# pweigmann/harmonic-power-flow

Measured on AMD Instinct MI355X. Metric: NR iterations/sec + ms/iter, 1 000-bus x 25-harmonic feeder; |dV| vs reference, higher is better.
Workload: dtype f64

## Files before the change

harmonic-power-flow_amd/csrc/hpf_block.hip:

```cpp
#include <algorithm>
#include <chrono>
#include <complex>
#include <cstdio>
#include <cstdlib>
#include <functional>
#include <rocsolver/rocsolver.h>
#include <thread>

#include "hpf_internal.hpp"
#include "hpf_gj.hpp"
#include "hpf_blk_jobs.hpp"
#include "hpf_blk_invert_mfma.hpp"
#include "hpf_gj_dense.hpp"
#include "hpf_gj_mfma.hpp"

using namespace hpf;

#ifdef HPF_FACTOR_STAMPS
#define HPF_STAMP_DECL long long st0 = 0, st1 = 0, st2 = 0, st3 = 0, st4 = 0, st5 = 0, st6 = 0
#define HPF_STAMP(v) \
    if (ablate & 16) v = __builtin_amdgcn_s_memtime()
#else
#define HPF_STAMP_DECL
#define HPF_STAMP(v)
// ... 676 lines not shown
                       h->cur_s0, h->d_pivflag, h->piv_limit, ts);
    return launch_status(h);
}

int wave_block_size(int b) { return b <= 12 ? 12 : (b <= 28 ? 28 : (b <= 52 ? 52 : (b <= 100 ? 100 : 0))); }

size_t factor_lds_bytes(int b) { return gj_dense_lds_bytes(b); }

template <int R>
int launch_factor(hpf_handle* h, const TreeDev& T, const int* nodes, int count, const int* active) {
    ScopedTimer t(h, T_SOLVE);
    const int b = 2 * h->Hn;
    const size_t lds = factor_lds_bytes(b);
    if (lds > 64 * 1024) {
        if (lds > 160 * 1024) return HPF_E_ARG;
        const hipError_t ea = hipFuncSetAttribute(reinterpret_cast<const void*>(&k_tree_factor<R>), hipFuncAttributeMaxDynamicSharedMemorySize, (int)lds);
        if (ea != hipSuccess) {
            h->last_detail = (int)ea;
            return HPF_E_HIP;
        }
    }
    hipLaunchKernelGGL((k_tree_factor<R>), dim3((unsigned)count, (unsigned)h->cur_S), dim3(256), lds, h->cur_stream, h->M, T,
                       nodes, b, h->N, h->Nc, active, h->d_U, h->d_E, h->d_f, h->d_Z, h->d_w, h->cur_s0);
    return launch_status(h);
}


template <int B>
__global__ __launch_bounds__(256) void k_level_back(
    Model M, TreeDev T, const int* __restrict__ sl_nodes, int n_sl, const int* __restrict__ lf_nodes, int n_lf, const int* __restrict__ gj_nodes, int n_gj,
    int b, int N, int Nc, const int* __restrict__ active, int S_cnt, const double* __restrict__ Zall, const double* __restrict__ wall,
    double* __restrict__ xall, const double* __restrict__ Hall, const double* __restrict__ Minv, const double* __restrict__ lbimg,
    const double* __restrict__ sbimg, const double* __restrict__ lzimg, const double* __restrict__ lfK, const double* __restrict__ lfS, int s0) {
    static_assert(64 * ((B + 16) / 16) == 256, "k_level_back: blocks of 52 rows (four wavefronts in every body)");
    const int ytiles = (S_cnt + LB_SB - 1) / LB_SB;
    const int bid = (int)blockIdx.x;
#if HPF_BATCH_XCD
    const int nb_sl = ((n_sl + 7) / 8) * 8 * ytiles, nb_lf = ((n_lf + 7) / 8) * 8 * ytiles;
    if (bid < nb_sl) {
        const int t_ = bid >> 3, bx = (t_ / ytiles) * 8 + (bid & 7);
        if (bx >= n_sl) return;
        sleaf_back_batch_body<B>(bx, t_ % ytiles, M, sl_nodes, b, active, S_cnt, wall, xall, Hall, sbimg, lzimg, Zall, lfS, s0);
    } else if (bid < nb_sl + nb_lf) {
        const int i = bid - nb_sl, t_ = i >> 3, bx = (t_ / ytiles) * 8 + (i & 7);
        if (bx >= n_lf) return;
        leaf_back_batch_body<B>(bx, t_ % ytiles, M, lf_nodes, b, active, S_cnt, wall, xall, Hall, lbimg, lfK, lfS, s0);
    } else {
#else
    const int nb_sl = n_sl * ytiles, nb_lf = n_lf * ytiles;
    if (bid < nb_sl) {
        sleaf_back_batch_body<B>(bid % n_sl, bid / n_sl, M, sl_nodes, b, active, S_cnt, wall, xall, Hall, sbimg, lzimg, Zall, lfS, s0);
    } else if (bid < nb_sl + nb_lf) {
        const int i = bid - nb_sl;
        leaf_back_batch_body<B>(i % n_lf, i / n_lf, M, lf_nodes, b, active, S_cnt, wall, xall, Hall, lbimg, lfK, lfS, s0);
    } else {
#endif
        const int i = bid - nb_sl - nb_lf;
        back_q_body<B>(i % n_gj, i / n_gj, M, T, gj_nodes, b, N, Nc, active, Zall, wall, xall, (double*)nullptr, Hall, Minv, lfK, lfS, s0);
    }
}

template <int B>
int launch_level_back(hpf_handle* h, const TreeDev& T, const int* sl_nodes, int n_sl, const int* lf_nodes, int n_lf, const int* gj_nodes, int n_gj,
                      const int* active) {
    const Tree& tr = active_tree(h);
    const unsigned ytiles = (unsigned)((h->cur_S + LB_SB - 1) / LB_SB);
#if HPF_BATCH_XCD
    const unsigned grid = (unsigned)(((n_sl + 7) / 8) * 8 + ((n_lf + 7) / 8) * 8) * ytiles + (unsigned)n_gj * (unsigned)h->cur_S;
#else
    const unsigned grid = (unsigned)(n_sl + n_lf) * ytiles + (unsigned)n_gj * (unsigned)h->cur_S;
#endif
    if ((unsigned)(n_sl + n_lf) * ytiles + (unsigned)n_gj * (unsigned)h->cur_S == 0) return HPF_OK;
    hipLaunchKernelGGL((k_level_back<B>), dim3(grid), dim3(256), 0, h->cur_stream, h->M, T, sl_nodes, n_sl, lf_nodes, n_lf, gj_nodes, n_gj, 2 * h->Hn,
                       h->N, h->Nc, active, h->cur_S, h->d_Z, h->d_w, h->d_x, h->d_H, tr.d_Minv, tr.d_lbimg, tr.d_sbimg, tr.d_lzimg, h->d_lfK, h->d_lfS,
                       h->cur_s0);
    return launch_status(h);
}

template <int B>
__global__ __launch_bounds__(64 * ((B + 16) / 16)) void k_back_walk(
    Model M, TreeDev T, const int* __restrict__ recs, const int* __restrict__ slots, const int* __restrict__ list_ptr, int b, int N, int Nc,
    const int* __restrict__ active, const double* __restrict__ Zall, const double* __restrict__ wall, double* __restrict__ xall,
    const double* __restrict__ Hall, const double* __restrict__ Minv, const double* __restrict__ lfK, const double* __restrict__ lfS, int s0) {
    __shared__ double xl[WALK_SLOTS + 2][B];
    const int beg = list_ptr[blockIdx.x], end = list_ptr[blockIdx.x + 1], tid = threadIdx.x;
    if (beg >= end) return;
    BackQIn<B> cur, nxt;
    back_q_load<B>(cur, beg, blockIdx.y, M, T, recs, b, active, Zall, wall, Hall, Minv, s0);
    if (cur.s < 0) return;
    const double* xs = xall + (size_t)cur.s * M.n * B;
    for (int i = beg; i < end; ++i) {
        const int2 sl = reinterpret_cast<const int2*>(slots)[i];
        const int par = cur.kp.y, crole = cur.kp.w >> 28;
        if (tid < B) {
            if (par >= 0 && sl.x < 0) xl[WALK_SLOTS][tid] = xs[(size_t)par * B + tid];
            if (crole == 1 && sl.y < 0) xl[WALK_SLOTS + 1][tid] = xs[(size_t)T.comp_child[cur.kp.w & 0x0fffffff] * B + tid];
        }
        lds_barrier();
        if (i + 1 < end) back_q_load<B>(nxt, i + 1, blockIdx.y, M, T, recs, b, active, Zall, wall, Hall, Minv, s0);
        const double x = back_q_compute<B>(cur, M, T, b, N, Nc, xall, (double*)nullptr, lfK, lfS, xl[sl.x < 0 ? WALK_SLOTS : sl.x],
                                           xl[sl.y < 0 ? WALK_SLOTS + 1 : sl.y]);
        if (tid < B) xl[(i - beg) % WALK_SLOTS][tid] = x;
        lds_barrier();
        cur = nxt;
    }
}

template <int B>
int launch_back_walk(hpf_handle* h, const Tree& tr, const TreeDev& T, int list0, int count, const int* active) {
    constexpr int NT = (B + 16) / 16;
    hipLaunchKernelGGL((k_back_walk<B>), dim3((unsigned)count, (unsigned)h->cur_S), dim3(64 * NT), 0, h->cur_stream, h->M, T, tr.d_walk_rec,
                       tr.d_walk_slot, tr.d_walk_ptr + list0, 2 * h->Hn, h->N, h->Nc, active, h->d_Z, h->d_w, h->d_x, h->d_H, tr.d_Minv,
                       h->d_lfK, h->d_lfS, h->cur_s0);
    return launch_status(h);
}

__global__ __launch_bounds__(256) void k_border_prepare(int n, int Hn, int Bst, int b, int r, int v0, int vfirst, const int* __restrict__ tb_bus,
                                                        int n_tb, const double* __restrict__ g, cplx* __restrict__ U, cplx* __restrict__ E,
                                                        cplx* __restrict__ I0, double* __restrict__ fb) {
    const int j = blockIdx.y, v = vfirst + j;
    const size_t dst = (size_t)(v0 + j);
    const int t = blockIdx.x * 256 + threadIdx.x;
    if (t < n * Hn) {
        U[dst * n * Hn + t] = U[(size_t)r * n * Hn + t];
        E[dst * n * Hn + t] = E[(size_t)r * n * Hn + t];
    }
    if (t < n) I0[dst * n + t] = I0[(size_t)r * n + t];
    if (t < n * Bst) {
        double val = 0.0;
        if (v == 0) {
            val = fb[(size_t)r * n * Bst + t];
            if (g) {
                const int bus = t / Bst, l = t - bus * Bst;
                if (l < b)
                    for (int a = 0; a < n_tb; ++a)
                        if (tb_bus[a] == bus) val -= g[a * b + l];
            }
        } else {
            const int a = (v - 1) / b, l = (v - 1) - a * b;
            if (t == tb_bus[a] * Bst + l) val = 1.0;
        }
        fb[dst * n * Bst + t] = val;
    }
}

__global__ __launch_bounds__(256) void k_border_build(Model M, int Bst, int b, int r, int v0, int vfirst, int m, const int* __restrict__ tb_bus,
                                                      const int* __restrict__ tb_ptr, const int* __restrict__ tb_adj,
                                                      const cplx* __restrict__ Uall, const cplx* __restrict__ Eall,
                                                      const double* __restrict__ xall, double* __restrict__ bM, double* __restrict__ brhs) {
    const int row = blockIdx.x * 256 + threadIdx.x;
    const int col = vfirst + blockIdx.y;
    if (row >= m) return;
    const int a = row / b, l = row - a * b, q = l >> 1, t = l & 1;
    const int i = tb_bus[a];
    const size_t so = (size_t)r * M.n * M.Hn;
    const double* x = xall + (size_t)(v0 + blockIdx.y) * M.n * Bst;
    double acc = 0.0;
    for (int e = tb_ptr[a]; e < tb_ptr[a + 1]; ++e) {
        const int j = tb_adj[3 * e], ent = tb_adj[3 * e + 1];
        double g4[4];
        coupling_block(M, Uall + so, Eall + so, q, i, j, ent, g4);
        acc = fma(g4[t * 2], x[(size_t)j * Bst + 2 * q], acc);
        acc = fma(g4[t * 2 + 1], x[(size_t)j * Bst + 2 * q + 1], acc);
    }
    if (col == 0)
        brhs[row] = acc;
    else
        bM[(size_t)(col - 1) * m + row] = acc + (row == col - 1 ? 1.0 : 0.0);
}

__global__ __launch_bounds__(256) void k_border_finish(int count, int r, int v0, int nv, double* __restrict__ xall, int* __restrict__ pivflag) {
    const int t = blockIdx.x * 256 + threadIdx.x;
    if (t < count) xall[(size_t)r * count + t] = xall[(size_t)v0 * count + t];
    if (t < nv && pivflag[v0 + t]) {
        atomicOr(pivflag + r, pivflag[v0 + t]);
        pivflag[v0 + t] = 0;
    }
}

}

#include "hpf_tree_plan.hpp"

namespace hpf {

static int level_batched(const hpf_handle* h, const Tree& T, int l, int* kind) {
    int nbatch = (l == 0 && h->sw.leafbatch && h->has_ctree && T.lvl_all_leaf[0]) ? T.n_lazy_level0 : 0;
// ... 986 lines not shown
```

harmonic-power-flow_amd/csrc/hpf_internal.hpp:

```cpp
#pragma once
#include <hip/hip_runtime.h>
#include <rocblas/rocblas.h>
#include <stdint.h>

#include <stdlib.h>
#include <string.h>

#include <string>
#include <vector>

#include "../../include/hpf.h"
#include "hpf_assembly.hpp"
#include "hpf_devmem.hpp"
#include "hpf_switches.hpp"

namespace hpf {

struct HipBackend {
    static constexpr int oom = (int)hipErrorOutOfMemory;
    static int alloc(void** p, size_t bytes) { return (int)hipMalloc(p, bytes); }
    static int free(void* p) { return (int)hipFree(p); }
    static int copy_in(void* dst, const void* src, size_t bytes) { return (int)hipMemcpy(dst, src, bytes, hipMemcpyHostToDevice); }
};
using DevMem = DevOwner<HipBackend>;

enum LinForm {
    LIN_ROOTS = 0,
    LIN_BUNDLE,
    LIN_TREE,
    LIN_LEVELS
};

enum { T_MISMATCH = 0, T_JACOBIAN = 1, T_SOLVE = 2, T_UPDATE = 3, T_BACK = 4, T_GJ = 5, T_GJ_DEV = 6, T_RESID = 7, T_COUNT = 8 };

struct TimedSpan {
    int which;
    hipEvent_t e0, e1;
};

#ifndef HPF_WALK_SLOTS
#define HPF_WALK_SLOTS 32
#endif
constexpr int WALK_LISTS = 8, WALK_SLOTS = HPF_WALK_SLOTS;
static_assert(WALK_SLOTS >= 2, "the walk's ring holds at least the previous bus");
constexpr int TAIL_SLOTS = 2;

struct Tree {
    int n_levels = 0;
    int n_depths = 0;
    std::vector<int> parent;
    std::vector<int> lvl_ptr;
    std::vector<int> lvl_nodes;
    std::vector<int> dep_ptr;
    std::vector<int> dep_nodes;
    std::vector<int> child_ptr;
    std::vector<int> child;
    std::vector<int> child_mid;
    std::vector<int> lin;
    std::vector<int> lin_ptr;
    std::vector<int> lin_post;
    std::vector<int> all_ptr, all_post;
    int n_lin_roots = 0;
    int n_dense = 0;
    int* d_parent = nullptr;
    int* d_lvl_nodes = nullptr;
    int* d_dep_nodes = nullptr;
    int* d_child_ptr = nullptr;
    int* d_child = nullptr;
    int* d_e_up = nullptr;
    int* d_e_dn = nullptr;
    int* d_child_mid = nullptr;
    int* d_lin = nullptr;
    int* d_lin_ptr = nullptr;
    int* d_lin_post = nullptr;
    int* d_all_ptr = nullptr;
    int* d_all_post = nullptr;
    int* d_fdesc = nullptr;
    int* d_child3 = nullptr;
    int* d_bdesc = nullptr;
    int n_chains = 0;
    std::vector<int> chain_ptr, chain_nodes, chain_ch;
    int* d_dchild = nullptr;
    int* d_chain_ptr = nullptr;
    int* d_chain_nodes = nullptr;
    int* d_chain_ch = nullptr;
    int n_lin_heights = 0;
    std::vector<int> lh_ptr;
    int* d_lrec = nullptr;
    int n_lin_bundles2 = 0, lin_np = 0;
    int lin_maxunit = 0;
    int* d_lb2rec = nullptr;
    int* d_lb2x = nullptr;
    int* d_lb2ptr = nullptr;
    int chains_bundled = 0;
    int* d_lb2cptr = nullptr;
    int* d_lb2clist = nullptr;
    int n_lin_bundles = 0;
    LinForm lin_form = LIN_ROOTS;
    bool chain_launches = false;
    int* d_lbrec = nullptr;
    int* d_lbptr = nullptr;
    int* d_crec = nullptr;
    int* d_cnode = nullptr;
    int n_all_heights = 0;
    std::vector<int> ah_ptr;
    int* d_arec = nullptr;
    std::vector<int> lvl_all_leaf;
    std::vector<int> toff_tab;
    std::vector<char> plain_gj;
    int n_cleaf = 0;
    double* d_Minv = nullptr;
    int n_lazy_parents = 0, n_lazy_leaves = 0;
    int n_lazy_level0 = 0;
    std::vector<int> lvl_nbatch;
    std::vector<int> dep_nleaf;
    std::vector<int> dep_nskip;
    int census[8] = {0, 0, 0, 0, 0, 0, 0, 0};
    std::vector<int> bsleaf_ptr;
    int n_bsleaf = 0;
    int* d_bsleaf = nullptr;
    double* d_sbimg = nullptr;
    std::vector<int> bsl_dep_ptr, bleaf_dep_ptr;
    int* d_bsleaf_dep = nullptr;
    int n_bleaf = 0;
    int* d_bleaf = nullptr;
    double* d_lbimg = nullptr;
    int* d_lzrec = nullptr;
// ... 252 lines not shown
```

harmonic-power-flow_amd/csrc/hpf_quad.hpp:

```cpp
#pragma once

template <int CTRL>
__device__ __forceinline__ double dpp_f64(double v) {
    int lo = __double2loint(v), hi = __double2hiint(v);
    lo = __builtin_amdgcn_update_dpp(lo, lo, CTRL, 0xf, 0xf, false);
    hi = __builtin_amdgcn_update_dpp(hi, hi, CTRL, 0xf, 0xf, false);
    return __hiloint2double(hi, lo);
}

__device__ __forceinline__ double row_sum16(double v) {
    v += dpp_f64<0xB1>(v);
    v += dpp_f64<0x4E>(v);
    v += dpp_f64<0x141>(v);
    v += dpp_f64<0x140>(v);
    return v;
}

__device__ __forceinline__ Blk2 blk_current(cplx y, cplx Uj, cplx Ej) {
    Blk2 b;
    b.dV = cmul_unf(y, Ej);
    b.dA = cmul_unf(cmulj(y), Uj);
    return b;
}
__device__ __forceinline__ Blk2 blk_current_diag(cplx y, cplx U, cplx E, cplx yn, bool nonlinear) {
    Blk2 b = blk_current(y, U, E);
    if (nonlinear) {
        b.dV = csub(b.dV, cmul_unf(yn, E));
        b.dA = csub(b.dA, cmul_unf(cmulj(yn), U));
    }
    return b;
}
__device__ __forceinline__ Blk2 blk_power_off(cplx y, cplx Ui, cplx Uj, cplx Ej) {
    const cplx yu = cmul_unf(y, Uj);
    const cplx ye = cmul_unf(y, Ej);
    Blk2 b;
    b.dV = cmul_unf(Ui, cconj(ye));
    b.dA = cmul_unf(cmulj(Ui), cconj(cneg(yu)));
    return b;
}
__device__ __forceinline__ Blk2 blk_power_diag(cplx y, cplx U, cplx E, cplx I) {
    const cplx yu = cmul_unf(y, U);
    const cplx ye = cmul_unf(y, E);
    Blk2 b;
    b.dV = cadd(cmul_unf(E, cconj(I)), cmul_unf(U, cconj(ye)));
    b.dA = cmul_unf(cmulj(U), cconj(csub(I, yu)));
    return b;
}
__device__ __forceinline__ void mask_block(int n, int c, int q, int i, int j, const Blk2& blk, double out[4]) {
#pragma unroll
    for (int tr = 0; tr < 2; ++tr)
#pragma unroll
        for (int tc = 0; tc < 2; ++tc)
            out[tr * 2 + tc] = (loc_valid(n, c, i, 2 * q + tr) && loc_valid(n, c, j, 2 * q + tc)) ? pick(blk, tr, tc) : 0.0;
}

template <int B>
struct TileIO {
    static constexpr int NT = (B + 16) / 16;
    static constexpr int LW = (B + 1 - 16 * (NT - 1)) <= 8 ? 8 : 16;
    static constexpr int RG = (NT - 1) * 64 + 4 * LW;
    static constexpr int NE = B / 4, NP = NE / 2;
    static_assert(NE == 2 * NP + 1, "odd number of row groups");
    __device__ static __forceinline__ size_t off2(int p, int wv, int lg, int jj) {
        return (size_t)p * 2 * RG + (wv < NT - 1 ? wv * 128 + (lg * 16 + jj) * 2 : (NT - 1) * 128 + (lg * LW + jj) * 2);
    }
    __device__ static __forceinline__ size_t off1(int wv, int lg, int jj) {
        return (size_t)NP * 2 * RG + (wv < NT - 1 ? wv * 64 + lg * 16 + jj : (NT - 1) * 64 + lg * LW + jj);
    }
    __device__ static __forceinline__ size_t off(int tr, int reg, int wv, int lg, int jj) {
        const int e = tr * 4 + reg;
        return e < 2 * NP ? off2(e >> 1, wv, lg, jj) + (e & 1) : off1(wv, lg, jj);
    }
    __device__ static __forceinline__ bool ok(int wv, int jj) { return wv < NT - 1 || jj < LW; }
    __device__ static __forceinline__ void load(const double* base, int wv, int lg, int jj, double (&v)[NT * 4]) {
        const bool in = ok(wv, jj);
#pragma unroll
        for (int p = 0; p < NP; ++p) {
            double2 t = {0.0, 0.0};
            if (in) t = *reinterpret_cast<const double2*>(base + off2(p, wv, lg, jj));
            v[2 * p] = t.x;
            v[2 * p + 1] = t.y;
        }
        v[NE - 1] = in ? base[off1(wv, lg, jj)] : 0.0;
    }
    __device__ static __forceinline__ void store(double* base, int wv, int lg, int jj, const double (&v)[NT * 4]) {
        if (!ok(wv, jj)) return;
#pragma unroll
        for (int p = 0; p < NP; ++p) *reinterpret_cast<double2*>(base + off2(p, wv, lg, jj)) = double2{v[2 * p], v[2 * p + 1]};
        base[off1(wv, lg, jj)] = v[NE - 1];
    }
};

template <int NT>
__device__ __forceinline__ void lz_aop(const double* p, double (&a)[NT]) {
    if constexpr (NT % 2 == 0) {
#pragma unroll
        for (int t2 = 0; t2 < NT / 2; ++t2) {
            const double2 v = *reinterpret_cast<const double2*>(p + 2 * t2);
            a[2 * t2] = v.x;
            a[2 * t2 + 1] = v.y;
        }
    } else {
#pragma unroll
        for (int t = 0; t < NT; ++t) a[t] = p[t];
    }
}

#define HPF_WAVE_LDS_FENCE() asm volatile("s_waitcnt lgkmcnt(0)" ::: "memory")

#ifndef HPF_LEAF_XCD
#define HPF_LEAF_XCD 1
#endif
#ifndef HPF_Q100L_OCC
#define HPF_Q100L_OCC 2
#endif
#ifndef HPF_Q100_OCC
#define HPF_Q100_OCC 2
#endif
#ifndef HPF_Q_OCC
#define HPF_Q_OCC 4
#endif

template <int B>
struct FqLds {
    static constexpr int NT = (B + 16) / 16, RP = 16 * NT > 64 ? 16 * NT : 64;
    cplx* ynl;
    double* tab;
    double* dgb;
    double (*cc)[RP * 3];
    double (*panel)[NT * 64];
    double (*wl)[16];
    double (*pv)[16];
    double* gl;
    double* hl;
    double* slb;
    double* gl2;
    double* hl2;
    double* pbuf;
    __device__ __forceinline__ static FqLds carve(double* smem_) {
        FqLds L;
        L.ynl = reinterpret_cast<cplx*>(smem_);
        L.tab = smem_ + 2 * (B / 2) * (B / 2);
        L.dgb = L.tab + (B / 2) * 8;
        L.cc = reinterpret_cast<double (*)[RP * 3]>(L.dgb + RP * 3);
        L.panel = reinterpret_cast<double (*)[NT * 64]>(L.dgb + RP * 3 + NT * RP * 3);
        L.wl = reinterpret_cast<double (*)[16]>(L.dgb + RP * 3 + NT * RP * 3 + 2 * NT * 64);
        L.pv = reinterpret_cast<double (*)[16]>(L.dgb + RP * 3 + NT * RP * 3 + 2 * NT * 64 + 32);
        L.gl = L.dgb + RP * 3 + NT * RP * 3 + 2 * NT * 64 + 64;
        L.hl = L.gl + NT * 32;
        L.slb = L.hl + NT * 32;
        L.gl2 = B <= 52 ? L.slb : L.slb + 2;
        L.hl2 = L.gl2 + NT * 32;
        L.pbuf = smem_;
        return L;
    }
};

template <int B>
constexpr int factor_q_lds() {
    constexpr int NT = (B + 16) / 16, RP = 16 * NT > 64 ? 16 * NT : 64;
    return (B / 2) * 8 + RP * 3 + NT * RP * 3 + 2 * NT * 64 + 32 + 32 + NT * 32 + NT * 32 + 2 * (B / 2) * (B / 2) +
           (B <= 52 ? 2 * B * 10 + 200 + 4 : 2 + 2 * NT * 32);
}
static_assert(factor_q_lds<52>() >= 52 * 53 && factor_q_lds<28>() >= 28 * 29 && factor_q_lds<12>() >= 12 * 13 && factor_q_lds<100>() >= 64 * 101,
              "dense-push buffer of a compress step fits the factor body's LDS");

// ... 1131 lines not shown
    double* __restrict__ lfK, double* __restrict__ lfS, long long* __restrict__ dbg, int ablate, int s0,
    int* __restrict__ pivflag, double piv_limit, unsigned long long* __restrict__ tstamp, int leaf_count, unsigned leaf_S) {
    constexpr int NT = (B + 16) / 16, RP = 16 * NT > 64 ? 16 * NT : 64;
    FqLds<B> lds;
    if constexpr (LEAF) {
        __shared__ cplx ynl[(B / 2) * (B / 2)];
        __shared__ double tab[(B / 2) * 8], dgb[RP * 3], cc[NT][RP * 3], panel[2][NT * 64], wl[2][16], pv[2][16], gl[NT * 32], hl[NT * 32];
        __shared__ double slb[B <= 52 ? 2 * B * 10 + 200 + 4 : 1];
        lds.ynl = ynl; lds.tab = tab; lds.dgb = dgb; lds.cc = cc; lds.panel = panel; lds.wl = wl; lds.pv = pv; lds.gl = gl; lds.hl = hl; lds.slb = slb;
        lds.gl2 = lds.hl2 = lds.pbuf = nullptr;
    } else {
        __shared__ __attribute__((aligned(16))) double smem[factor_q_lds<B>()];
        lds = FqLds<B>::carve(smem);
    }
    int bx = blockIdx.x, by = blockIdx.y;
#if HPF_LEAF_XCD
    if constexpr (LEAF) {
        const unsigned id = blockIdx.x, t = id >> 3, S_ = gridDim.y == 1 ? leaf_S : 1u;
        by = (int)(t % S_);
        bx = (int)((t / S_) * 8u + (id & 7u));
        if (bx >= leaf_count) return;
    }
#endif
    factor_q_body<B, LEAF>(lds, bx, by, M, T, nodes, b, N, Nc, active, Uall, Eall, fall, Zall, wall, linAall, Call, Hall, I0all, chG,
                           chH, chD, chy, Minv, lfK, lfS, dbg, ablate, s0, pivflag, piv_limit, tstamp);
}

__device__ __forceinline__ void lds_barrier() {
    __builtin_amdgcn_fence(__ATOMIC_RELEASE, "workgroup", "local");
    __builtin_amdgcn_s_barrier();
    __builtin_amdgcn_fence(__ATOMIC_ACQUIRE, "workgroup", "local");
}

template <int B>
struct BackQIn {
    static constexpr int NT = (B + 16) / 16;
    int4 kp;
    int s;
    double x;
    double zr[NT * 4];
    double hk0, hk1, h20, h21;
};

template <int B>
__device__ __forceinline__ void back_q_load(
    BackQIn<B>& in, const int bx_, const int by_, const Model& M, const TreeDev& T, const int* __restrict__ nodes, int b,
    const int* __restrict__ active, const double* __restrict__ Zall, const double* __restrict__ wall, const double* __restrict__ Hall,
    const double* __restrict__ Minv, int s0) {
    constexpr int NT = (B + 16) / 16;
    constexpr size_t CT = (size_t)NT * NT * 256;
    const int s = active ? active[by_ + s0] : (int)by_ + s0;
    in.s = s;
    if (s < 0) return;
    const int4 kp = reinterpret_cast<const int4*>(nodes)[bx_];
    in.kp = kp;
    const int k = kp.x, par = kp.y, cleaf = kp.z;
    const int crole = kp.w >> 28, cinfo = kp.w & 0x0fffffff;
    const int tid = threadIdx.x, lane = tid & 63, lg = lane >> 4, jj = lane & 15;
    const int wv = __builtin_amdgcn_readfirstlane(tid >> 6);
    const int n = M.n, Hn = M.Hn;
    in.x = 0.0;
    if (tid < B) in.x = wall[((size_t)s * n + k) * B + tid];
    if (par >= 0) {
        if (cleaf) {
            TileIO<B>::load(Minv + (size_t)(cleaf - 1) * CT, wv, lg, jj, in.zr);
        } else {
            TileIO<B>::load(Zall + ((size_t)s * n + k) * CT, wv, lg, jj, in.zr);
        }
        const int col = 16 * wv + jj, p = col >> 1, t1 = col & 1;
        if (crole != 2 && col < b) {
            const double* hk = Hall + ((size_t)s * n + k) * Hn * 4 + p * 4 + t1 * 2;
            in.hk0 = hk[0];
            in.hk1 = hk[1];
            if (crole == 1) {
                const double* h2 = T.cH2 + ((size_t)s * T.n_comp + cinfo) * Hn * 4 + p * 4 + t1 * 2;
                in.h20 = h2[0];
                in.h21 = h2[1];
            }
        }
    }
}

template <int B>
__device__ __forceinline__ double back_q_compute(
    const BackQIn<B>& in, const Model& M, const TreeDev& T, int b, int N, int Nc, double* __restrict__ xall, double* __restrict__ step,
    const double* __restrict__ lfK, const double* __restrict__ lfS, const double* xp, const double* xc) {
    constexpr int NT = (B + 16) / 16;
    constexpr size_t CT = (size_t)NT * NT * 256;
    const int s = in.s;
    const int k = in.kp.x, par = in.kp.y, cleaf = in.kp.z;
    const int crole = in.kp.w >> 28, cinfo = in.kp.w & 0x0fffffff;
    const int tid = threadIdx.x, lane = tid & 63, lg = lane >> 4, jj = lane & 15;
    const int wv = __builtin_amdgcn_readfirstlane(tid >> 6);
    const int n = M.n, c = M.c, Hn = M.Hn;
    double* xs = xall + (size_t)s * n * B;
    constexpr int RP = 16 * NT > 64 ? 16 * NT : 64;
    __shared__ double part[NT][RP];
    __shared__ double mcl[RP * 2], zl[RP];
    double x = in.x;
    if (par >= 0) {
        const int col = 16 * wv + jj, p = col >> 1, t1 = col & 1;
        double tv = 0.0;
        if (crole == 2) {
            double hr[NT * 4];
            TileIO<B>::load(T.cF + (((size_t)s * T.n_comp + cinfo) * 3 + 2) * CT, wv, lg, jj, hr);
            const double xpc = col < b ? xp[col] : 0.0;
#pragma unroll
            for (int e = 0; e < NT * 4; ++e)
                if (16 * (e >> 2) + 4 * (e & 3) < B) {
                    const double r = row_sum16(hr[e] * xpc);
                    if (jj == 0) part[wv][16 * (e >> 2) + lg + 4 * (e & 3)] = r;
                }
            lds_barrier();
            if (tid < B) {
                double acc = part[0][tid];
#pragma unroll
                for (int w2 = 1; w2 < NT; ++w2) acc += part[w2][tid];
                zl[tid] = acc;
            }
            lds_barrier();
            tv = col < b ? zl[col] : 0.0;
            lds_barrier();
        } else if (col < b) {
            tv = fma(in.hk1, xp[2 * p + 1], in.hk0 * xp[2 * p]);
            if (crole == 1) tv += fma(in.h21, xc[2 * p + 1], in.h20 * xc[2 * p]);
        }
        if (cleaf && tid < 2) zl[tid] = tv;
        const double tvs = (cleaf && col < 2) ? 0.0 : tv;
        __builtin_amdgcn_sched_barrier(0);
#pragma unroll
        for (int e = 0; e < NT * 4; ++e)
            if (16 * (e >> 2) + 4 * (e & 3) < B) {
                const double r = row_sum16(in.zr[e] * tvs);
                if (jj == 0) part[wv][16 * (e >> 2) + lg + 4 * (e & 3)] = r;
                if (cleaf && wv == 0 && jj < 2) mcl[(16 * (e >> 2) + lg + 4 * (e & 3)) * 2 + jj] = in.zr[e];
            }
        lds_barrier();
        double acc = 0.0;
        if (tid < B) {
            acc = part[0][tid];
#pragma unroll
            for (int w2 = 1; w2 < NT; ++w2) acc += part[w2][tid];
        }
        if (cleaf) {
            double t0 = 0.0, t1v = 0.0;
            if (tid < B) {
                t0 = zl[0];
                t1v = zl[1];
            }
            lds_barrier();
            if (tid < 2) zl[tid] = acc + (tid == 0 ? t0 : t1v);
            lds_barrier();
            if (tid < B) {
                const double* kk = lfK + ((size_t)s * n + k) * 12;
                const double u0 = fma(kk[1], zl[1], kk[0] * zl[0]), u1 = fma(kk[3], zl[1], kk[2] * zl[0]);
                const double c0r = tid < 2 ? (tid == 0 ? 1.0 : 0.0) : mcl[tid * 2];
                const double c1r = tid < 2 ? (tid == 1 ? 1.0 : 0.0) : mcl[tid * 2 + 1];
                acc = fma(c1r, u1, fma(c0r, u0, tid < 2 ? 0.0 : acc));
            }
            lds_barrier();
            if (tid < B) zl[tid] = acc;
            lds_barrier();
            if (tid < B) {
                const double* si = lfS + (((size_t)s * n + k) * Hn + (tid >> 1)) * 4 + 2 * (tid & 1);
                acc = (tid >> 1) < Hn ? fma(si[1], zl[tid | 1], si[0] * zl[tid & ~1]) : acc;
            }
        }
        if (tid < B) x -= acc;
    }
    if (tid < B) {
        xs[(size_t)k * B + tid] = x;
        if (step && tid < b) {
            const int kst = (tid >> 1) * n + k;
            double* st = step + (size_t)s * N;
            if (tid & 1) {
                if (kst >= c) st[Nc + kst - c] = x;
            } else {
                if (kst >= 1) st[kst - 1] = x;
            }
        }
    }
    return x;
}

template <int B>
__device__ __forceinline__ void back_q_body(
    const int bx_, const int by_, const Model& M, const TreeDev& T, const int* __restrict__ nodes, int b, int N, int Nc, const int* __restrict__ active,
    const double* __restrict__ Zall, const double* __restrict__ wall, double* __restrict__ xall, double* __restrict__ step,
    const double* __restrict__ Hall, const double* __restrict__ Minv, const double* __restrict__ lfK,
    const double* __restrict__ lfS, int s0) {
    BackQIn<B> in;
    back_q_load<B>(in, bx_, by_, M, T, nodes, b, active, Zall, wall, Hall, Minv, s0);
    if (in.s < 0) return;
    const double* xs = xall + (size_t)in.s * M.n * B;
    const int par = in.kp.y, crole = in.kp.w >> 28;
    const double* xp = par >= 0 ? xs + (size_t)par * B : nullptr;
    const double* xc = crole == 1 ? xs + (size_t)T.comp_child[in.kp.w & 0x0fffffff] * B : nullptr;
    back_q_compute<B>(in, M, T, b, N, Nc, xall, step, lfK, lfS, xp, xc);
}

template <int B>
__global__ __launch_bounds__(64 * ((B + 16) / 16)) void k_back_q(
    Model M, TreeDev T, const int* __restrict__ nodes, int b, int N, int Nc, const int* __restrict__ active,
    const double* __restrict__ Zall, const double* __restrict__ wall, double* __restrict__ xall, double* __restrict__ step,
    const double* __restrict__ Hall, const double* __restrict__ Minv, const double* __restrict__ lfK,
    const double* __restrict__ lfS, int s0) {
    back_q_body<B>(blockIdx.x, blockIdx.y, M, T, nodes, b, N, Nc, active, Zall, wall, xall, step, Hall, Minv, lfK, lfS, s0);
}

template <int B, bool LEAF>
int launch_factor_q2(hpf_handle* h, const TreeDev& T, const int* nodes, int count, const int* active) {
    ScopedTimer t(h, LEAF ? T_SOLVE : T_GJ);
    unsigned long long* ts = nullptr;
    if (!LEAF && h->timing && h->d_tstamp && h->ts_next < hpf_handle::TS_CAP) ts = h->d_tstamp + 2 * (size_t)(h->ts_next++);
    constexpr int NT = (B + 16) / 16;
    dim3 grid((unsigned)count, (unsigned)h->cur_S);
#if HPF_LEAF_XCD
    if (LEAF) grid = dim3((unsigned)(((count + 7) / 8) * 8) * (unsigned)h->cur_S, 1, 1);
#endif
// ... 21 lines not shown
```

Before: 153,800.

## Pipeline back-walk operand loads across register sets with LDS-staged records

Reworks the serial back-substitution walk kernel to keep several buses' operands in rotating register sets, issuing loads a configurable depth ahead. Walk records and slot pairs are staged in LDS in chunks and read as wave-uniform scalars. The compound-node H tile is prefetched mid-compute through a callback, and the extra barrier is skipped when no parent x reload is needed. This targets global-load latency on the sequential dependency chain, at the cost of higher register pressure and more complex control flow. With the default depth of 1, the pipeline still double-buffers.

```diff
diff --git a/harmonic-power-flow_amd/csrc/hpf_block.hip b/harmonic-power-flow_amd/csrc/hpf_block.hip
--- a/harmonic-power-flow_amd/csrc/hpf_block.hip
+++ b/harmonic-power-flow_amd/csrc/hpf_block.hip
@@ -782,27 +782,117 @@
     Model M, TreeDev T, const int* __restrict__ recs, const int* __restrict__ slots, const int* __restrict__ list_ptr, int b, int N, int Nc,
     const int* __restrict__ active, const double* __restrict__ Zall, const double* __restrict__ wall, double* __restrict__ xall,
     const double* __restrict__ Hall, const double* __restrict__ Minv, const double* __restrict__ lfK, const double* __restrict__ lfS, int s0) {
+    constexpr int NT = (B + 16) / 16, NS = WALK_SETS, D = WALK_DEPTH, CH = WALK_CHUNK;
+    static_assert(2 * CH <= 64 * NT, "one thread per staged record");
     __shared__ double xl[WALK_SLOTS + 2][B];
+    __shared__ int4 recl[2 * CH];
+    __shared__ int2 slotl[2 * CH];
     const int beg = list_ptr[blockIdx.x], end = list_ptr[blockIdx.x + 1], tid = threadIdx.x;
-    if (beg >= end) return;
-    BackQIn<B> cur, nxt;
-    back_q_load<B>(cur, beg, blockIdx.y, M, T, recs, b, active, Zall, wall, Hall, Minv, s0);
-    if (cur.s < 0) return;
-    const double* xs = xall + (size_t)cur.s * M.n * B;
-    for (int i = beg; i < end; ++i) {
-        const int2 sl = reinterpret_cast<const int2*>(slots)[i];
+    const int s = active ? active[blockIdx.y + s0] : (int)blockIdx.y + s0;
+    if (beg >= end || s < 0) return;
+    const int len = end - beg, lane = tid & 63, jj = lane & 15;
+    const int wv = __builtin_amdgcn_readfirstlane(tid >> 6);
+    const int4* rec4 = reinterpret_cast<const int4*>(recs) + beg;
+    const int2* slot2 = reinterpret_cast<const int2*>(slots) + beg;
+    if (tid < 2 * CH && tid < len) {
+        recl[tid] = rec4[tid];
+        slotl[tid] = slot2[tid];
+    }
+    __syncthreads();
+    const double* xs = xall + (size_t)s * M.n * B;
+    BackQIn<B> in[NS];
+    int2 sl[NS];
+    double hd[NT * 4];
+    int4 nrec = {0, 0, 0, 0};
+    int2 nslot = {0, 0};
+#pragma unroll
+    for (int e = 0; e < NT * 4; ++e) hd[e] = 0.0;
+    auto record = [&](int j, int4& kp, int2& s2) {
+        const int q = (j < len ? j : len - 1) % (2 * CH);
+        const int4 r = recl[q];
+        const int2 t = slotl[q];
+        kp = int4{__builtin_amdgcn_readfirstlane(r.x), __builtin_amdgcn_readfirstlane(r.y), __builtin_amdgcn_readfirstlane(r.z),
+                  __builtin_amdgcn_readfirstlane(r.w)};
+        s2 = int2{__builtin_amdgcn_readfirstlane(t.x), __builtin_amdgcn_readfirstlane(t.y)};
+    };
+    auto fetch = [&](auto uc, int j) {
+        constexpr int U = decltype(uc)::value;
+        int4 kp;
+        record(j, kp, sl[U]);
+        back_walk_load<B>(in[U], kp, s, M, T, b, Zall, Hall, Minv);
+    };
+    {
+        int4 kp0;
+        int2 t0;
+        record(0, kp0, t0);
+        if ((kp0.w >> 28) == 2) back_walk_load_hd<B>(hd, kp0, s, T);
+    }
+    fetch(std::integral_constant<int, 0>{}, 0);
+    back_walk_load_w<B>(in[0], M, wall);
+    if constexpr (D >= 2) {
+        fetch(std::integral_constant<int, 1 % NS>{}, 1);
+        back_walk_load_w<B>(in[1 % NS], M, wall);
+    }
+    if constexpr (D >= 3) {
+        fetch(std::integral_constant<int, 2 % NS>{}, 2);
+        back_walk_load_w<B>(in[2 % NS], M, wall);
+    }
+    if constexpr (D >= 4) {
+        fetch(std::integral_constant<int, 3 % NS>{}, 3);
+        back_walk_load_w<B>(in[3 % NS], M, wall);
+    }
+    auto bus = [&](auto uc, auto fc, const int j) {
+        constexpr int U = decltype(uc)::value, UN = (U + 1) % NS, UF = (U + D) % NS;
+        constexpr bool FETCH = decltype(fc)::value;
+        BackQIn<B>& cur = in[U];
+        const int2 s2 = sl[U];
         const int par = cur.kp.y, crole = cur.kp.w >> 28;
-        if (tid < B) {
-            if (par >= 0 && sl.x < 0) xl[WALK_SLOTS][tid] = xs[(size_t)par * B + tid];
-            if (crole == 1 && sl.y < 0) xl[WALK_SLOTS + 1][tid] = xs[(size_t)T.comp_child[cur.kp.w & 0x0fffffff] * B + tid];
+        if ((par >= 0 && s2.x < 0) || (crole == 1 && s2.y < 0)) {
+            if (tid < B) {
+                if (par >= 0 && s2.x < 0) xl[WALK_SLOTS][tid] = xs[(size_t)par * B + tid];
+                if (crole == 1 && s2.y < 0) xl[WALK_SLOTS + 1][tid] = xs[(size_t)T.comp_child[cur.kp.w & 0x0fffffff] * B + tid];
+            }
+            lds_barrier();
+        }
+        if constexpr (FETCH && D < NS) fetch(std::integral_constant<int, UF>{}, j + D);
+        auto refill = [&]() {
+            if (j + 1 < len && (in[UN].kp.w >> 28) == 2) back_walk_load_hd<B>(hd, in[UN].kp, s, T);
+            if constexpr (FETCH && D == NS) fetch(std::integral_constant<int, UF>{}, j + D);
+        };
+        TileIO<B>::zero_outside(wv, jj, cur.zr);
+        if (crole == 2) TileIO<B>::zero_outside(wv, jj, hd);
+        const double x = back_q_compute<B>(cur, M, T, b, N, Nc, xall, (double*)nullptr, lfK, lfS, xl[s2.x < 0 ? WALK_SLOTS : s2.x],
+                                           xl[s2.y < 0 ? WALK_SLOTS + 1 : s2.y], hd, refill);
+        if (tid < B) xl[j % WALK_SLOTS][tid] = x;
+        if constexpr (FETCH) {
+            back_walk_load_w<B>(in[UF], M, wall);
+            if (j % CH == 0 && j >= CH && tid < CH && j + CH + tid < len) {
+                nrec = rec4[j + CH + tid];
+                nslot = slot2[j + CH + tid];
+            }
+            if (j % CH == CH / 2 && j > CH && tid < CH && j + CH / 2 + tid < len) {
+                recl[(j + CH / 2 + tid) % (2 * CH)] = nrec;
+                slotl[(j + CH / 2 + tid) % (2 * CH)] = nslot;
+            }
         }
         lds_barrier();
-        if (i + 1 < end) back_q_load<B>(nxt, i + 1, blockIdx.y, M, T, recs, b, active, Zall, wall, Hall, Minv, s0);
-        const double x = back_q_compute<B>(cur, M, T, b, N, Nc, xall, (double*)nullptr, lfK, lfS, xl[sl.x < 0 ? WALK_SLOTS : sl.x],
-                                           xl[sl.y < 0 ? WALK_SLOTS + 1 : sl.y]);
-        if (tid < B) xl[(i - beg) % WALK_SLOTS][tid] = x;
-        lds_barrier();
-        cur = nxt;
+    };
+    constexpr std::true_type loop{};
+    constexpr std::false_type rest{};
+    int j = 0;
+    for (; j + NS <= len; j += NS) {
+        bus(std::integral_constant<int, 0>{}, loop, j);
+        bus(std::integral_constant<int, 1>{}, loop, j + 1);
+        if constexpr (NS >= 3) bus(std::integral_constant<int, 2 % NS>{}, loop, j + 2);
+        if constexpr (NS >= 4) bus(std::integral_constant<int, 3 % NS>{}, loop, j + 3);
+    }
+    if (j < len) {
+        bus(std::integral_constant<int, 0>{}, rest, j);
+        if (j + 1 < len) {
+            bus(std::integral_constant<int, 1>{}, rest, j + 1);
+            if constexpr (NS >= 4)
+                if (j + 2 < len) bus(std::integral_constant<int, 2 % NS>{}, rest, j + 2);
+        }
     }
 }
 
diff --git a/harmonic-power-flow_amd/csrc/hpf_internal.hpp b/harmonic-power-flow_amd/csrc/hpf_internal.hpp
--- a/harmonic-power-flow_amd/csrc/hpf_internal.hpp
+++ b/harmonic-power-flow_amd/csrc/hpf_internal.hpp
@@ -43,6 +43,14 @@
 #endif
 constexpr int WALK_LISTS = 8, WALK_SLOTS = HPF_WALK_SLOTS;
 static_assert(WALK_SLOTS >= 2, "the walk's ring holds at least the previous bus");
+#ifndef HPF_WALK_DEPTH
+#define HPF_WALK_DEPTH 1
+#endif
+constexpr int WALK_DEPTH = HPF_WALK_DEPTH, WALK_SETS = WALK_DEPTH == 1 ? 2 : WALK_DEPTH;
+static_assert(HPF_WALK_DEPTH >= 1 && HPF_WALK_DEPTH <= 4, "k_back_walk names its register sets: four at most");
+static_assert(HPF_WALK_DEPTH < WALK_SLOTS, "the operands in flight belong to buses whose x the ring will still hold");
+constexpr int WALK_CHUNK = 16;
+static_assert(WALK_CHUNK % 2 == 0 && WALK_CHUNK / 2 > 4, "a chunk's refill is written half a chunk after its request, ahead of the deepest prefetch");
 constexpr int TAIL_SLOTS = 2;
 
 struct Tree {
diff --git a/harmonic-power-flow_amd/csrc/hpf_quad.hpp b/harmonic-power-flow_amd/csrc/hpf_quad.hpp
--- a/harmonic-power-flow_amd/csrc/hpf_quad.hpp
+++ b/harmonic-power-flow_amd/csrc/hpf_quad.hpp
@@ -82,6 +82,21 @@
             v[2 * p + 1] = t.y;
         }
         v[NE - 1] = in ? base[off1(wv, lg, jj)] : 0.0;
+    }
+    __device__ static __forceinline__ void load_all(const double* base, int wv, int lg, int jj, double (&v)[NT * 4]) {
+        const int j2 = ok(wv, jj) ? jj : (jj & (LW - 1));
+#pragma unroll
+        for (int p = 0; p < NP; ++p) {
+            const double2 t = *reinterpret_cast<const double2*>(base + off2(p, wv, lg, j2));
+            v[2 * p] = t.x;
+            v[2 * p + 1] = t.y;
+        }
+        v[NE - 1] = base[off1(wv, lg, j2)];
+    }
+    __device__ static __forceinline__ void zero_outside(int wv, int jj, double (&v)[NT * 4]) {
+        const bool in = ok(wv, jj);
+#pragma unroll
+        for (int e = 0; e < NE; ++e) v[e] = in ? v[e] : 0.0;
     }
     __device__ static __forceinline__ void store(double* base, int wv, int lg, int jj, const double (&v)[NT * 4]) {
         if (!ok(wv, jj)) return;
@@ -1379,9 +1394,62 @@
 }
 
 template <int B>
+__device__ __forceinline__ void back_walk_load(
+    BackQIn<B>& in, const int4 kp, const int s, const Model& M, const TreeDev& T, int b, const double* __restrict__ Zall,
+    const double* __restrict__ Hall, const double* __restrict__ Minv) {
+    constexpr int NT = (B + 16) / 16;
+    constexpr size_t CT = (size_t)NT * NT * 256;
+    in.s = s;
+    in.kp = kp;
+    const int k = kp.x, cleaf = kp.z;
+    const int crole = kp.w >> 28, cinfo = kp.w & 0x0fffffff;
+    const int tid = threadIdx.x, lane = tid & 63, lg = lane >> 4, jj = lane & 15;
+    const int wv = __builtin_amdgcn_readfirstlane(tid >> 6);
+    const int n = M.n, Hn = M.Hn;
+    const size_t sk = (size_t)s * n + k;
+    TileIO<B>::load_all(cleaf ? Minv + (size_t)(cleaf - 1) * CT : Zall + sk * CT, wv, lg, jj, in.zr);
+    const int col = 16 * wv + jj, colc = col < b ? col : 0, p = colc >> 1, t1 = colc & 1;
+    const double* hk = Hall + sk * Hn * 4 + p * 4 + t1 * 2;
+    const double* h2 = crole == 1 ? T.cH2 + ((size_t)s * T.n_comp + cinfo) * Hn * 4 + p * 4 + t1 * 2 : hk;
+    in.hk0 = hk[0];
+    in.hk1 = hk[1];
+    in.h20 = h2[0];
+    in.h21 = h2[1];
+}
+
+template <int B>
+__device__ __forceinline__ void back_walk_load_w(BackQIn<B>& in, const Model& M, const double* __restrict__ wall) {
+    const int tid = threadIdx.x;
+    in.x = wall[((size_t)in.s * M.n + in.kp.x) * B + (tid < B ? tid : 0)];
+}
+
+template <int B>
+__device__ __forceinline__ void back_walk_load_hd(double (&hd)[((B + 16) / 16) * 4], const int4 kp, const int s, const TreeDev& T) {
+    constexpr int NT = (B + 16) / 16;
+    constexpr size_t CT = (size_t)NT * NT * 256;
+    const int tid = threadIdx.x, lane = tid & 63, lg = lane >> 4, jj = lane & 15;
+    const int wv = __builtin_amdgcn_readfirstlane(tid >> 6);
+    TileIO<B>::load_all(T.cF + (((size_t)s * T.n_comp + (kp.w & 0x0fffffff)) * 3 + 2) * CT, wv, lg, jj, hd);
+}
+
+template <int B>
+__device__ __forceinline__ void back_q_lds(double (*&part)[16 * ((B + 16) / 16) > 64 ? 16 * ((B + 16) / 16) : 64], double*& mcl, double*& zl) {
+    constexpr int NT = (B + 16) / 16, RP = 16 * NT > 64 ? 16 * NT : 64;
+    __shared__ double part_[NT][RP];
+    __shared__ double mcl_[RP * 2], zl_[RP];
+    part = part_;
+    mcl = mcl_;
+    zl = zl_;
+}
+
+struct BackQNoMid {
+    __device__ __forceinline__ void operator()() const {}
+};
+
+template <int B, class Mid = BackQNoMid>
 __device__ __forceinline__ double back_q_compute(
     const BackQIn<B>& in, const Model& M, const TreeDev& T, int b, int N, int Nc, double* __restrict__ xall, double* __restrict__ step,
-    const double* __restrict__ lfK, const double* __restrict__ lfS, const double* xp, const double* xc) {
+    const double* __restrict__ lfK, const double* __restrict__ lfS, const double* xp, const double* xc, const double* hd = nullptr, Mid mid = Mid()) {
     constexpr int NT = (B + 16) / 16;
     constexpr size_t CT = (size_t)NT * NT * 256;
     const int s = in.s;
@@ -1392,15 +1460,20 @@
     const int n = M.n, c = M.c, Hn = M.Hn;
     double* xs = xall + (size_t)s * n * B;
     constexpr int RP = 16 * NT > 64 ? 16 * NT : 64;
-    __shared__ double part[NT][RP];
-    __shared__ double mcl[RP * 2], zl[RP];
+    double(*part)[RP], *mcl, *zl;
+    back_q_lds<B>(part, mcl, zl);
     double x = in.x;
     if (par >= 0) {
         const int col = 16 * wv + jj, p = col >> 1, t1 = col & 1;
         double tv = 0.0;
         if (crole == 2) {
             double hr[NT * 4];
-            TileIO<B>::load(T.cF + (((size_t)s * T.n_comp + cinfo) * 3 + 2) * CT, wv, lg, jj, hr);
+            if (hd) {
+#pragma unroll
+                for (int e = 0; e < NT * 4; ++e) hr[e] = hd[e];
+            } else {
+                TileIO<B>::load(T.cF + (((size_t)s * T.n_comp + cinfo) * 3 + 2) * CT, wv, lg, jj, hr);
+            }
             const double xpc = col < b ? xp[col] : 0.0;
 #pragma unroll
             for (int e = 0; e < NT * 4; ++e)
@@ -1432,6 +1505,9 @@
                 if (jj == 0) part[wv][16 * (e >> 2) + lg + 4 * (e & 3)] = r;
                 if (cleaf && wv == 0 && jj < 2) mcl[(16 * (e >> 2) + lg + 4 * (e & 3)) * 2 + jj] = in.zr[e];
             }
+    }
+    mid();
+    if (par >= 0) {
         lds_barrier();
         double acc = 0.0;
         if (tid < B) {
```

Result: no change. 155,300 (median of 3 runs) (+1.0%).
